# DRL-Navigation/DDRL4NAV

Hardware: AMD Instinct MI355X
Metric: env-steps/sec (whole node) + PPO update ms, Pong 256 envs at 1/2/4/8 GPUs (higher is better)
Workload: dtype f32 (f16x3 MFMA planes, fp32 accumulate)

## Files before the change

ddrl4nav_amd/csrc/common.h:

```cpp
#pragma once
#include <hip/hip_runtime.h>
#include <stdint.h>

#include "../../include/ddrl.h"

namespace ddrl {

constexpr int IMG = 84;
constexpr int FEAT = 512;
constexpr int FLAT = 3136;
constexpr int C1_OC = 32, C1_KS = 8, C1_S = 4, C1_OW = 20, C1_P = 400;
constexpr int C2_IC = 32, C2_OC = 64, C2_KS = 4, C2_S = 2, C2_IW = 20, C2_OW = 9, C2_P = 81, C2_K = 512;
constexpr int C3_IC = 64, C3_OC = 64, C3_KS = 3, C3_S = 1, C3_IW = 9, C3_OW = 7, C3_P = 49, C3_K = 576;
constexpr float LEAKY = 0.01f;

struct EncLayout {
  int64_t c1w, c1b, c2w, c2b, c3w, c3b, lw, lb, size;
};
struct ParamLayout {
  int A, C;
  int NE;
  EncLayout enc;
  int64_t enc_base[2];
  int64_t actor_w, actor_b, critic_w, critic_b;
  int64_t n_params, n_actor;
};

inline ParamLayout make_layout(int A, int C, bool shared = false) {
  ParamLayout L;
  L.A = A;
  L.C = C;
  L.NE = shared ? 1 : 2;
  int64_t o = 0;
  L.enc.c1w = o; o += (int64_t)C1_OC * C * 64;
  L.enc.c1b = o; o += C1_OC;
  L.enc.c2w = o; o += (int64_t)C2_OC * C2_K;
  L.enc.c2b = o; o += C2_OC;
  L.enc.c3w = o; o += (int64_t)C3_OC * C3_K;
  L.enc.c3b = o; o += C3_OC;
  L.enc.lw = o; o += (int64_t)FEAT * FLAT;
  L.enc.lb = o; o += FEAT;
  L.enc.size = o;
  int64_t p = 0;
  L.enc_base[0] = p; p += L.enc.size;
  L.actor_w = p; p += (int64_t)A * FEAT;
  L.actor_b = p; p += A;
  L.n_actor = p;
  L.critic_w = p; p += FEAT;
  L.critic_b = p; p += 1;
  if (shared) {
    L.enc_base[1] = L.enc_base[0];
    L.n_params = p;
    L.n_actor = p;
    return L;
  }
  L.enc_base[1] = p; p += L.enc.size;
  L.n_params = p;
  return L;
}

struct Workspace {
  unsigned short* wp1b;
  unsigned short* wp2b;
  unsigned short* wp3b;
  unsigned short* wd2b;
  unsigned short* wd3b;
  unsigned short* wlb;
  unsigned short* wdlb;
  float* amax;
  float* actmax;
  float *a1, *a2, *a3, *h;
  unsigned* m1;
  unsigned* m2;
  unsigned* m3;
  float *dz1, *dz2, *dz3, *dh;
  float* gsc;
  float* dlogits;
  float* dvalue;
  float* wpart;
  int64_t wpart_floats;
  float* hpart;
  double* npart;
  float* lut;
  int64_t total_bytes;
};

constexpr int AMAX_WL = 0, AMAX_W2 = 1, AMAX_W3 = 2, AMAX_W1 = 3, AMAX_A1 = 4, AMAX_A2 = 5, AMAX_A3 = 6, AMAX_DH = 7, AMAX_DZ3 = 8,
              AMAX_DZ2 = 9, AMAX_DZ1 = 10, AMAX_GMAX = 11, AMAX_SLOTS = 12, AMAX_FIRST_ACT = AMAX_A2;
constexpr float WGRAD_HEADROOM = 4.0f;
constexpr int GSC_EXP_MIN = -60, GSC_EXP_MAX = 60;
__host__ __device__ inline int amax_idx(int slot, int e) { return slot * 2 + e; }
__host__ __device__ inline float f16_scale(float m) {
  if (!(m > 0.0f) || !(m < 3.0e38f)) return 1.0f;
  int e;
  frexpf(m, &e);
  return ldexpf(1.0f, 13 - e);
}
constexpr int HEAD_WG = 256;
constexpr int NORM_WG = 1024;

inline int64_t align_up(int64_t x, int64_t a) { return (x + a - 1) / a * a; }
__host__ __device__ inline int64_t m1_words(int64_t max_batch) { return max_batch * 400; }
__host__ __device__ inline int m1_bit(int oc) { return ((oc >> 2) & 1) * 16 + 15 - ((oc & 3) + 4 * (oc >> 3)); }

constexpr int ACT_FUSED_MAX = 512;
constexpr int FC_ACT_SPLITS = 14;
static_assert(FC_ACT_SPLITS > 1 && 98 % FC_ACT_SPLITS == 0, "FC_ACT_SPLITS: a divisor of 98 larger than 1");
struct Splits {
  int c1, c2, c3, fc;
};
inline Splits choose_splits(int max_batch, int NE = 2) {
  constexpr int C1_SPLITS = 512, C2_SPLITS = 256, C3_SPLITS = 256;
  const int pairs = (max_batch + 1) / 2;
  auto cap = [&](int want, int limit) { return want < limit ? (want < 1 ? 1 : want) : (limit < 1 ? 1 : limit); };
  Splits s;
  s.c1 = cap(C1_SPLITS, pairs);
  const int k = 2 / NE;
  s.c2 = cap(C2_SPLITS * k, pairs);
  s.c3 = cap(C3_SPLITS * k, pairs);
  s.fc = cap(5 * k, (max_batch + 31) / 32);
  return s;
}

inline int64_t hpart_stride(int A) { return align_up((int64_t)(A + 1) * FEAT + A + 1 + 4, 64); }

inline int64_t carve(Workspace& w, const ddrl_config& c, void* base) {
  const int64_t MB = c.max_batch, C = c.in_channels, A = c.n_actions;
  int64_t off = 0;
  auto take = [&](int64_t floats) -> float* {
    float* p = base ? (float*)((char*)base + off) : nullptr;
    off += align_up(floats * 4, 256);
    return p;
  };
  w.wp1b = (unsigned short*)take(4 * 4 * 3 * 2 * 64 * 8 / 2);
  w.wlb = (unsigned short*)take(2 * 3 * (int64_t)FLAT * FEAT / 2);
  w.wdlb = (unsigned short*)take(2 * 3 * (int64_t)FLAT * FEAT / 2);
  w.amax = take(64);
  w.actmax = take(2 * ACT_FUSED_MAX);
  w.wp2b = (unsigned short*)take(2 * 32 * 3 * 64 * 16 / 2);
  w.wp3b = (unsigned short*)take(2 * 8 * 5 * 3 * 64 * 16 / 2);
  w.wd2b = (unsigned short*)take(2 * 2 * 4 * 4 * 3 * 64 * 16 / 2);
  w.wd3b = (unsigned short*)take(2 * 8 * 5 * 3 * 64 * 16 / 2);
  w.a1 = take(2 * MB * 32 * 400);
  w.m1 = (unsigned*)take(2 * m1_words(MB));
  w.m2 = (unsigned*)take(2 * MB * 81 * 2);
  w.m3 = (unsigned*)take(2 * MB * 49 * 2);
  w.a2 = take(2 * MB * 64 * 81);
  w.a3 = take(2 * MB * FLAT);
  w.h = take(2 * MB * FEAT);
  w.dz1 = take(2 * MB * 32 * 400);
  w.dz2 = take(2 * MB * 64 * 81);
  w.dz3 = take(2 * MB * FLAT);
  w.dh = take(2 * MB * FEAT);
  w.gsc = take(2 * MB);
  w.dlogits = take(MB * A);
  w.dvalue = take(MB);
  Splits s = choose_splits(c.max_batch, c.share_cnn_net ? 1 : 2);
  int64_t p1 = (int64_t)s.c1 * 2 * (32 * C * 64 + 32);
  int64_t p2 = (int64_t)s.c2 * 2 * (64 * 512 + 64);
  int64_t p3 = (int64_t)s.c3 * 2 * (64 * 576 + 64);
  int64_t pf = (int64_t)s.fc * 2 * ((int64_t)FEAT * FLAT + FEAT);
  int64_t pm = p1;
  if (p2 > pm) pm = p2;
  if (p3 > pm) pm = p3;
  if (pf > pm) pm = pf;
  const int64_t pact = (int64_t)FC_ACT_SPLITS * 2 * (MB < 1024 ? MB : 1024) * FEAT;
  if (pact > pm) pm = pact;
  w.wpart_floats = pm;
  w.wpart = take(pm);
  w.hpart = take((int64_t)HEAD_WG * hpart_stride(A));
  w.npart = (double*)take(NORM_WG * 2);
  w.lut = take(256);
  w.total_bytes = off;
  return off;
}

__host__ __device__ inline uint64_t splitmix64(uint64_t x) {
  x += 0x9E3779B97F4A7C15ull;
  uint64_t z = x;
  z = (z ^ (z >> 30)) * 0xBF58476D1CE4E5B9ull;
  z = (z ^ (z >> 27)) * 0x94D049BB133111EBull;
  return z ^ (z >> 31);
}
__host__ __device__ inline float hash_uniform(uint64_t seed, uint64_t stream, uint64_t idx) {
  uint64_t base = splitmix64(splitmix64(seed) ^ stream);
  uint64_t z = splitmix64(base + idx);
  return (float)(z >> 40) * (1.0f / 16777216.0f);
}

}
```

ddrl4nav_amd/csrc/conv2.hip:

```cpp
#include "engine2.h"

namespace ddrl {


using u4v = __attribute__((ext_vector_type(4))) unsigned;

constexpr int F1_PITCH = 168;
template <int NE>
struct Fwd1B {
  static constexpr int ROWS = 32 * NE, A_BYTES = 4 * NPL * 2 * ROWS * 16, PITCH = F1_PITCH, IMG_BYTES = 64 * PITCH;
  static constexpr int STAGE_BYTES = A_BYTES + IMG_BYTES, AQ = A_BYTES / 16, NAJ = AQ / 256;
  static constexpr size_t LDS_BYTES = 2 * STAGE_BYTES;
};

template <int NE>
__global__ __launch_bounds__(256) void conv_fwd1_planes_kernel(const uint8_t* __restrict__ frames, const unsigned short* __restrict__ wp1b,
                                                               float* __restrict__ amax, const float* __restrict__ params, int64_t bias_off0,
                                                               int64_t bias_off1, float* __restrict__ out, int64_t out_es, int n,
                                                               unsigned* __restrict__ m1, int64_t m1_es, int C) {
  using K = Fwd1B<NE>;
  extern __shared__ __attribute__((aligned(16))) char ldsb[];
  const int tid = threadIdx.x, lane = tid & 63, wc = tid >> 6, l31 = lane & 31, hi = lane >> 5;
  const int c0 = blockIdx.x * 256, ctot = n * 400, clast = min(c0 + 255, ctot - 1);
  const int b0 = c0 / 400, b1 = clast / 400, oyf0 = (c0 % 400) / 20, iy0_start = 4 * oyf0;
// ... 289 lines not shown
                     w.wp1b, w.amax, c.params, L.enc_base[0] + L.enc.c1b, L.enc_base[NE - 1] + L.enc.c1b, w.a1, c.max_batch * 12800, c.n,
                     acting ? (unsigned*)nullptr : w.m1, m1_words(c.max_batch), L.C);
}

struct Fwd2B {
  static constexpr int SPT = 3, KC = 2;
  static constexpr int WPE = 3;
  static constexpr int ROW = 52, CH = 20 * ROW, IMG_PLANE = SPT * KC * CH;
  static constexpr int W_OFF = NPL * IMG_PLANE, W_BYTES = KC * NPL * 64 * 32;
  static constexpr int BIAS_OFF = W_OFF + W_BYTES;
  static constexpr int NIU = SPT * KC * 100, NIJ = (NIU + 255) / 256;
  static constexpr int NWJ = W_BYTES / 16 / 256;
  static constexpr int STAGE_BYTES = BIAS_OFF;
  static constexpr size_t LDS_BYTES = STAGE_BYTES + 64 * 4;
};
struct __attribute__((packed, aligned(4))) lds_u2 {
  unsigned x, y;
};

__global__ __launch_bounds__(256) __attribute__((amdgpu_waves_per_eu(Fwd2B::WPE, Fwd2B::WPE))) void conv_fwd2_planes_kernel(const float* __restrict__ a1, int64_t a1_es, const unsigned short* __restrict__ wp2b,
                                                               float* __restrict__ amax, const float* __restrict__ params, int64_t bias_off0,
                                                               int64_t bias_off1, float* __restrict__ out, int64_t out_es, int n,
                                                               unsigned* __restrict__ m2) {
  using K = Fwd2B;
  extern __shared__ __attribute__((aligned(16))) char ldsc2[];
  const int tid = threadIdx.x, lane = tid & 63, wc = tid >> 6, l31 = lane & 31, hi = lane >> 5;
  const int e = blockIdx.z, b0 = blockIdx.x * K::SPT;
  const float sa = plane_scale(amax[amax_idx(AMAX_A1, e)]), inv = 1.0f / (sa * plane_scale(amax[amax_idx(AMAX_W2, e)]));
  if (tid < 64) ((float*)(ldsc2 + K::STAGE_BYTES))[tid] = params[(e ? bias_off1 : bias_off0) + tid];
  const float* isrc[K::NIJ];
  int idst[K::NIJ];
#pragma unroll
  for (int j = 0; j < K::NIJ; ++j) {
    const int u = min(tid + 256 * j, K::NIU - 1);
    const int s = u / (100 * K::KC), rem = u % (100 * K::KC), q = rem % 100;
    isrc[j] = a1 + e * a1_es + (int64_t)min(b0 + s, n - 1) * 12800 + rem * 4;
    idst[j] = (s * K::KC + rem / 100) * K::CH + (q / 5) * K::ROW + (q % 5) * 8;
  }
  const unsigned short* wsrc = wp2b + (int64_t)e * (32 * NPL * 64 * 16) + tid * 8;
  int aA[2], bB[2];
#pragma unroll
  for (int i = 0; i < 2; ++i) aA[i] = K::W_OFF + (i * 32 + l31) * 32 + hi * 16;
#pragma unroll
  for (int j = 0; j < 2; ++j) {
    int c = wc * 64 + j * 32 + l31;
    if (c >= K::SPT * 81) c = 0;
    const int s = c / 81, pix = c % 81, oy = pix / 9, ox = pix % 9;
    bB[j] = s * K::KC * K::CH + (2 * oy + 2 * hi) * K::ROW + 4 * ox;
  }
  f4 ir[K::NIJ], wr[K::NWJ];
  auto fetch = [&](int kb) {
#pragma unroll
    for (int j = 0; j < K::NIJ; ++j) ir[j] = ld4(isrc[j] + kb * (400 * K::KC));
#pragma unroll
    for (int j = 0; j < K::NWJ; ++j) wr[j] = *(const f4*)(wsrc + kb * (K::KC * NPL * 1024) + j * 2048);
  };
  auto commit = [&](char* ldsc2) {
#pragma unroll
    for (int j = 0; j < K::NIJ; ++j) {
      if (j + 1 < K::NIJ || tid + 256 * j < K::NIU) {
        const f4 v = ir[j];
        unsigned pa[NPL], pb[NPL];
        split_planes(v.x, v.y, sa, pa);
        split_planes(v.z, v.w, sa, pb);
        char* d = ldsc2 + idst[j];
#pragma unroll
        for (int p = 0; p < NPL; ++p) *(lds_u2*)(d + p * K::IMG_PLANE) = lds_u2{pa[p], pb[p]};
      }
    }
#pragma unroll
    for (int j = 0; j < K::NWJ; ++j) *(f4*)(ldsc2 + K::W_OFF + (tid + 256 * j) * 16) = wr[j];
  };
  f32x16 acc[2][2];
#pragma unroll
  for (int i = 0; i < 2; ++i)
#pragma unroll
    for (int j = 0; j < 2; ++j)
#pragma unroll
      for (int r = 0; r < 16; ++r) acc[i][j][r] = 0.0f;
  constexpr int NKB = 32 / K::KC;
  auto compute = [&](const char* ldsc2) {
#pragma unroll
    for (int kg = 0; kg < K::KC; ++kg) {
      frag8 a[NPL][2], b[NPL][2];
#pragma unroll
      for (int p = 0; p < NPL; ++p) {
#pragma unroll
        for (int i = 0; i < 2; ++i) a[p][i] = *(const frag8*)(ldsc2 + aA[i] + (kg * NPL + p) * 2048);
#pragma unroll
        for (int j = 0; j < 2; ++j) {
          const char* q = ldsc2 + bB[j] + p * K::IMG_PLANE + kg * K::CH;
          const lds_u2 lo = *(const lds_u2*)q, up = *(const lds_u2*)(q + K::ROW);
          b[p][j] = __builtin_bit_cast(frag8, (u4v){lo.x, lo.y, up.x, up.y});
        }
      }
#pragma unroll
      for (int t = 0; t < NPROD; ++t)
#pragma unroll
        for (int i = 0; i < 2; ++i)
#pragma unroll
          for (int j = 0; j < 2; ++j) acc[i][j] = mfma_planes(a[PA[t]][i], b[PB[t]][j], acc[i][j]);
    }
  };
  fetch(0);
  commit(ldsc2);
  fetch(1);
  __syncthreads();
  for (int kb = 0; kb < NKB; ++kb) {
    compute(ldsc2);
    __syncthreads();
    if (kb + 1 < NKB) {
      commit(ldsc2);
      if (kb + 2 < NKB) fetch(kb + 2);
    }
    __syncthreads();
  }
  const float* bias = (const float*)(ldsc2 + K::STAGE_BYTES);
  float big = 0.0f;
#pragma unroll
  for (int j = 0; j < 2; ++j) {
    const int c = wc * 64 + j * 32 + l31;
    const int s = c / 81, pix = c % 81;
    if (c >= K::SPT * 81 || b0 + s >= n) continue;
    float* base = out + e * out_es + (int64_t)b0 * 5184;
    const uint32_t lb = (uint32_t)((s * 5184 + pix + hi * (4 * 81)) * 4);
    unsigned bits = 0u;
#pragma unroll
    for (int i = 0; i < 2; ++i)
#pragma unroll
      for (int r = 0; r < 16; ++r) {
        const int oc = i * 32 + acc_row(r, hi);
        const float y = leaky_f(__builtin_fmaf(acc[i][j][r], inv, bias[oc]));
        st1_so(base + (i * 32 + acc_row(r, 0)) * 81, lb, y);
        big = fmaxf(big, fabsf(y));
        bits = __builtin_amdgcn_alignbit(bits, (unsigned)__builtin_elementwise_sub_sat((int)__float_as_uint(y), 1), 31);
      }
    if (m2 != nullptr) m2[(e * (out_es / 5184) + b0 + s) * 162 + pix * 2 + hi] = (bits >> 16) | (bits << 16);
  }
  amax_update(big, amax + amax_idx(AMAX_A2, e));
}
static void launch_fwd2_planes(const EncCall& c, bool acting, hipStream_t st) {
  using K = Fwd2B;
  const Workspace& w = *c.ws;
  const ParamLayout& L = *c.L;
  lds_limit_once<conv_fwd2_planes_kernel>((int)K::LDS_BYTES);
  hipLaunchKernelGGL(conv_fwd2_planes_kernel, dim3((unsigned)((c.n + K::SPT - 1) / K::SPT), 1, (unsigned)L.NE), dim3(256), K::LDS_BYTES, st, w.a1,
                     c.max_batch * 12800, w.wp2b, w.amax, c.params, L.enc_base[0] + L.enc.c2b, L.enc_base[L.NE - 1] + L.enc.c2b, w.a2, c.max_batch * 5184,
                     c.n, acting ? (unsigned*)nullptr : w.m2);
}

struct Fwd3B {
  static constexpr int WPE = 3;
  static constexpr int TN = 2, SPT = (128 * TN) / 49, NPX = SPT * 81;
  static constexpr int IMG_PLANE = NPX * 16;
  static constexpr int W_OFF = NPL * IMG_PLANE, W_BYTES = 5 * NPL * 64 * 32;
  static constexpr int BIAS_OFF = W_OFF + W_BYTES;
  static constexpr int NIJ = (NPX + 255) / 256;
  static constexpr int NWJ = (W_BYTES / 16 + 255) / 256;
  static constexpr size_t LDS_BYTES = BIAS_OFF + 64 * 4;
};

__global__ __launch_bounds__(256) __attribute__((amdgpu_waves_per_eu(Fwd3B::WPE, Fwd3B::WPE))) void conv_fwd3_planes_kernel(const float* __restrict__ a2, int64_t a2_es, const unsigned short* __restrict__ wp3b,
                                                               float* __restrict__ amax, const float* __restrict__ params, int64_t bias_off0,
                                                               int64_t bias_off1, float* __restrict__ out, int64_t out_es, int n,
                                                               unsigned* __restrict__ m3) {
  using K = Fwd3B;
  extern __shared__ __attribute__((aligned(16))) char ldsc3[];
  const int tid = threadIdx.x, lane = tid & 63, wc = tid >> 6, l31 = lane & 31, hi = lane >> 5;
  const int e = blockIdx.z, b0 = blockIdx.x * K::SPT;
  const float sa = plane_scale(amax[amax_idx(AMAX_A2, e)]), inv = 1.0f / (sa * plane_scale(amax[amax_idx(AMAX_W3, e)]));
  if (tid < 64) ((float*)(ldsc3 + K::BIAS_OFF))[tid] = params[(e ? bias_off1 : bias_off0) + tid];
  const float* isrc[K::NIJ];
#pragma unroll
  for (int j = 0; j < K::NIJ; ++j) {
    const int u = min(tid + 256 * j, K::NPX - 1);
    const int s = u / 81, px = u % 81;
    isrc[j] = a2 + e * a2_es + (int64_t)min(b0 + s, n - 1) * 5184 + px;
  }
  const unsigned short* wsrc = wp3b + (int64_t)e * (8 * 5 * NPL * 64 * 16) + tid * 8;
  int aA[2], bB[K::TN], tapoff[5];
#pragma unroll
  for (int i = 0; i < 2; ++i) aA[i] = K::W_OFF + (i * 32 + l31) * 32 + hi * 16;
#pragma unroll
  for (int j = 0; j < K::TN; ++j) {
    int c = wc * (32 * K::TN) + j * 32 + l31;
    if (c >= K::SPT * 49) c = 0;
    const int s = c / 49, pix = c % 49;
    bB[j] = (s * 81 + (pix / 7) * 9 + pix % 7) * 16;
  }
#pragma unroll
  for (int kg = 0; kg < 5; ++kg) {
    const int tap = min(2 * kg + hi, 8);
    tapoff[kg] = ((tap / 3) * 9 + tap % 3) * 16;
  }
  float ir[K::NIJ][8];
  f4 wr[K::NWJ];
  auto fetch = [&](int kb) {
#pragma unroll
    for (int j = 0; j < K::NIJ; ++j)
#pragma unroll
      for (int c = 0; c < 8; ++c) ir[j][c] = isrc[j][(kb * 8 + c) * 81];
#pragma unroll
    for (int j = 0; j < K::NWJ; ++j)
      if (j + 1 < K::NWJ || tid + 256 * j < K::W_BYTES / 16) wr[j] = *(const f4*)(wsrc + kb * (5 * NPL * 1024) + j * 2048);
  };
  auto commit = [&]() {
#pragma unroll
    for (int j = 0; j < K::NIJ; ++j) {
      if (j + 1 < K::NIJ || tid + 256 * j < K::NPX) {
        unsigned pl[4][NPL];
#pragma unroll
        for (int c = 0; c < 4; ++c) split_planes(ir[j][2 * c], ir[j][2 * c + 1], sa, pl[c]);
        char* d = ldsc3 + (tid + 256 * j) * 16;
#pragma unroll
        for (int p = 0; p < NPL; ++p) *(u4v*)(d + p * K::IMG_PLANE) = (u4v){pl[0][p], pl[1][p], pl[2][p], pl[3][p]};
      }
    }
#pragma unroll
    for (int j = 0; j < K::NWJ; ++j)
      if (j + 1 < K::NWJ || tid + 256 * j < K::W_BYTES / 16) *(f4*)(ldsc3 + K::W_OFF + (tid + 256 * j) * 16) = wr[j];
  };
  f32x16 acc[2][K::TN];
#pragma unroll
  for (int i = 0; i < 2; ++i)
#pragma unroll
    for (int j = 0; j < K::TN; ++j)
#pragma unroll
      for (int r = 0; r < 16; ++r) acc[i][j][r] = 0.0f;
  constexpr int NKB = 8;
  fetch(0);
  commit();
  fetch(1);
  __syncthreads();
  for (int kb = 0; kb < NKB; ++kb) {
#pragma unroll
    for (int kg = 0; kg < 5; ++kg) {
      frag8 a[NPL][2], b[NPL][K::TN];
#pragma unroll
      for (int p = 0; p < NPL; ++p) {
#pragma unroll
        for (int i = 0; i < 2; ++i) a[p][i] = *(const frag8*)(ldsc3 + aA[i] + (kg * NPL + p) * 2048);
#pragma unroll
        for (int j = 0; j < K::TN; ++j) b[p][j] = *(const frag8*)(ldsc3 + bB[j] + tapoff[kg] + p * K::IMG_PLANE);
      }
#pragma unroll
      for (int t = 0; t < NPROD; ++t)
#pragma unroll
        for (int i = 0; i < 2; ++i)
#pragma unroll
          for (int j = 0; j < K::TN; ++j) acc[i][j] = mfma_planes(a[PA[t]][i], b[PB[t]][j], acc[i][j]);
    }
    __syncthreads();
    if (kb + 1 < NKB) {
      commit();
      if (kb + 2 < NKB) fetch(kb + 2);
    }
    __syncthreads();
  }
  const float* bias = (const float*)(ldsc3 + K::BIAS_OFF);
  float big = 0.0f;
#pragma unroll
  for (int j = 0; j < K::TN; ++j) {
    const int c = wc * (32 * K::TN) + j * 32 + l31;
    const int s = c / 49, pix = c % 49;
    if (c >= K::SPT * 49 || b0 + s >= n) continue;
    float* base = out + e * out_es + (int64_t)b0 * FLAT;
    const uint32_t lb = (uint32_t)((s * FLAT + pix + hi * (4 * 49)) * 4);
    unsigned bits = 0u;
#pragma unroll
    for (int i = 0; i < 2; ++i)
#pragma unroll
      for (int r = 0; r < 16; ++r) {
        const int oc = i * 32 + acc_row(r, hi);
        const float y = leaky_f(__builtin_fmaf(acc[i][j][r], inv, bias[oc]));
        st1_so(base + (i * 32 + acc_row(r, 0)) * 49, lb, y);
        big = fmaxf(big, fabsf(y));
        bits = __builtin_amdgcn_alignbit(bits, (unsigned)__builtin_elementwise_sub_sat((int)__float_as_uint(y), 1), 31);
      }
    if (m3 != nullptr) m3[(e * (out_es / FLAT) + b0 + s) * 98 + pix * 2 + hi] = (bits >> 16) | (bits << 16);
  }
  amax_update(big, amax + amax_idx(AMAX_A3, e));
}
static void launch_fwd3_planes(const EncCall& c, bool acting, hipStream_t st) {
  using K = Fwd3B;
  const Workspace& w = *c.ws;
  const ParamLayout& L = *c.L;
  lds_limit_once<conv_fwd3_planes_kernel>((int)K::LDS_BYTES);
  hipLaunchKernelGGL(conv_fwd3_planes_kernel, dim3((unsigned)((c.n + K::SPT - 1) / K::SPT), 1, (unsigned)L.NE), dim3(256), K::LDS_BYTES, st, w.a2,
                     c.max_batch * 5184, w.wp3b, w.amax, c.params, L.enc_base[0] + L.enc.c3b, L.enc_base[L.NE - 1] + L.enc.c3b, w.a3, c.max_batch * FLAT,
                     c.n, acting ? (unsigned*)nullptr : w.m3);
}


void launch_conv_forward2(const EncCall& c, bool acting, hipStream_t st) {
  {
    ProfRange pr(c.prof, acting ? "ConvFwd1.act" : "ConvFwd1", st);
    if (c.L->NE == 2) {
      launch_fwd1_planes<2>(c, acting, st);
    } else {
      launch_fwd1_planes<1>(c, acting, st);
    }
  }
  {
    ProfRange pr(c.prof, acting ? "ConvFwd2.act" : "ConvFwd2", st);
    launch_fwd2_planes(c, acting, st);
  }
  {
    ProfRange pr(c.prof, acting ? "ConvFwd3.act" : "ConvFwd3", st);
    launch_fwd3_planes(c, acting, st);
  }
}

struct Dgrad3B {
  static constexpr int THREADS = 256, TN = 2, SPT = ((THREADS / 64) * 32 * TN) / 81;
  static constexpr int KOC = 16, NKB = 64 / KOC, PIXB = 2 * KOC;
  static constexpr int IMG_PLANE = SPT * 121 * PIXB;
  static constexpr int W_OFF = NPL * IMG_PLANE, W_BYTES = 9 * NPL * 64 * 32;
  static constexpr int NIU = SPT * 49, NIJ = (NIU + THREADS - 1) / THREADS;
  static constexpr int NWQ = W_BYTES / 16, NWJ = (NWQ + THREADS - 1) / THREADS;
  static constexpr size_t LDS_BYTES = W_OFF + W_BYTES;
};

__global__ __launch_bounds__(Dgrad3B::THREADS) __attribute__((amdgpu_waves_per_eu(2, 2))) void conv_dgrad3_planes_kernel(
    const float* __restrict__ dz3, int64_t dz_es, const unsigned short* __restrict__ wd3b, float* __restrict__ amax, const unsigned* __restrict__ m2,
    float* __restrict__ out, int64_t out_es, int n) {
  using K = Dgrad3B;
  extern __shared__ __attribute__((aligned(16))) char ldsd3[];
  const int tid = threadIdx.x, lane = tid & 63, wc = tid >> 6, l31 = lane & 31, hi = lane >> 5;
  const int e = blockIdx.z, b0 = blockIdx.x * K::SPT;
  const float sa = plane_scale(amax[amax_idx(AMAX_DZ3, e)]), inv = 1.0f / (sa * plane_scale(amax[amax_idx(AMAX_W3, e)]));
  for (int i = tid; i < K::W_OFF / 16; i += K::THREADS) *(f4*)(ldsd3 + i * 16) = zero4();
  const float* isrc[K::NIJ];
  int idst[K::NIJ];
#pragma unroll
  for (int j = 0; j < K::NIJ; ++j) {
    const int u = min(tid + K::THREADS * j, K::NIU - 1);
    const int s = u / 49, px = u % 49;
    isrc[j] = dz3 + e * dz_es + (int64_t)min(b0 + s, n - 1) * FLAT + px;
    idst[j] = (s * 121 + (px / 7 + 2) * 11 + px % 7 + 2) * K::PIXB;
  }
  const unsigned short* wsrc = wd3b + (int64_t)e * (K::NKB * 9 * NPL * 64 * 16) + tid * 8;
  int aA[2], bB[K::TN];
#pragma unroll
  for (int i = 0; i < 2; ++i) aA[i] = K::W_OFF + (i * 32 + l31) * 32 + hi * 16;
#pragma unroll
  for (int j = 0; j < K::TN; ++j) {
    int c = wc * (32 * K::TN) + j * 32 + l31;
    if (c >= K::SPT * 81) c = 0;
    const int s = c / 81, pix = c % 81;
    bB[j] = (s * 121 + (pix / 9 + 2) * 11 + pix % 9 + 2) * K::PIXB + hi * 16;
  }
  float ir[K::NIJ][K::KOC];
  f4 wr[K::NWJ];
  auto fetch = [&](int kb) {
#pragma unroll
    for (int j = 0; j < K::NIJ; ++j)
#pragma unroll
      for (int c = 0; c < K::KOC; ++c) ir[j][c] = isrc[j][(kb * K::KOC + c) * 49];
#pragma unroll
    for (int j = 0; j < K::NWJ; ++j)
      if (j + 1 < K::NWJ || tid + K::THREADS * j < K::NWQ) wr[j] = *(const f4*)(wsrc + kb * (9 * NPL * 1024) + j * (K::THREADS * 8));
  };
  auto commit = [&]() {
#pragma unroll
    for (int j = 0; j < K::NIJ; ++j) {
      if (j + 1 < K::NIJ || tid + K::THREADS * j < K::NIU) {
        unsigned pl[K::KOC / 2][NPL];
#pragma unroll
        for (int c = 0; c < K::KOC / 2; ++c) split_planes(ir[j][2 * c], ir[j][2 * c + 1], sa, pl[c]);
        char* d = ldsd3 + idst[j];
#pragma unroll
        for (int p = 0; p < NPL; ++p) {
          *(u4v*)(d + p * K::IMG_PLANE) = (u4v){pl[0][p], pl[1][p], pl[2][p], pl[3][p]};
          *(u4v*)(d + p * K::IMG_PLANE + 16) = (u4v){pl[4][p], pl[5][p], pl[6][p], pl[7][p]};
        }
      }
    }
#pragma unroll
    for (int j = 0; j < K::NWJ; ++j)
      if (j + 1 < K::NWJ || tid + K::THREADS * j < K::NWQ) *(f4*)(ldsd3 + K::W_OFF + (tid + K::THREADS * j) * 16) = wr[j];
  };
  f32x16 acc[2][K::TN];
#pragma unroll
  for (int i = 0; i < 2; ++i)
#pragma unroll
    for (int j = 0; j < K::TN; ++j)
#pragma unroll
      for (int r = 0; r < 16; ++r) acc[i][j][r] = 0.0f;
  fetch(0);
  __syncthreads();
  commit();
  fetch(1);
  __syncthreads();
  for (int kb = 0; kb < K::NKB; ++kb) {
#pragma unroll
    for (int t = 0; t < 9; ++t) {
      constexpr int ROW11 = 11;
      const int toff = ((t / 3) * ROW11 + t % 3) * K::PIXB;
      frag8 af[NPL][2], bfr[NPL][K::TN];
#pragma unroll
      for (int p = 0; p < NPL; ++p) {
#pragma unroll
        for (int i = 0; i < 2; ++i) af[p][i] = *(const frag8*)(ldsd3 + aA[i] + (t * NPL + p) * 2048);
#pragma unroll
        for (int j = 0; j < K::TN; ++j) bfr[p][j] = *(const frag8*)(ldsd3 + bB[j] - toff + p * K::IMG_PLANE);
      }
#pragma unroll
      for (int m = 0; m < NPROD; ++m)
#pragma unroll
        for (int i = 0; i < 2; ++i)
#pragma unroll
          for (int j = 0; j < K::TN; ++j) acc[i][j] = mfma_planes(af[PA[m]][i], bfr[PB[m]][j], acc[i][j]);
    }
    __syncthreads();
    if (kb + 1 < K::NKB) {
      commit();
      if (kb + 2 < K::NKB) fetch(kb + 2);
    }
    __syncthreads();
  }
  float big = 0.0f;
#pragma unroll
  for (int j = 0; j < K::TN; ++j) {
    const int c = wc * (32 * K::TN) + j * 32 + l31;
    const int s = c / 81, pix = c % 81;
    if (c >= K::SPT * 81 || b0 + s >= n) continue;
    const int64_t off = (int64_t)(b0 + s) * 5184 + pix + hi * (4 * 81);
    float* op = out + e * out_es + off;
    const unsigned mw = m2[(e * (out_es / 5184) + b0 + s) * 162 + pix * 2 + hi];
#pragma unroll
    for (int i = 0; i < 2; ++i)
#pragma unroll
      for (int r = 0; r < 16; ++r) {
        const float g = leaky_bit(mw, 16 * i + 15 - r, acc[i][j][r] * inv);
        op[(i * 32 + acc_row(r, 0)) * 81] = g;
        big = fmaxf(big, fabsf(g));
      }
  }
  amax_update(big, amax + amax_idx(AMAX_DZ2, e));
}
static void launch_dgrad3_planes(const EncCall& c, hipStream_t st) {
  using K = Dgrad3B;
// ... 137 lines not shown
```

ddrl4nav_amd/csrc/optim.hip:

```cpp
#include "engine2.h"

namespace ddrl {

__device__ __forceinline__ void pack_conv1_planes_body(const float* __restrict__ params, const ParamLayout& L, unsigned short* __restrict__ dst,
                                                       const float* __restrict__ amax, int bx) {
  const int rows = 32 * L.NE;
  const int idx = bx * 256 + threadIdx.x;
  if (idx >= L.C * 4 * 2 * rows * 8) return;
  const int j = idx & 7, row = (idx >> 3) % rows, r = (idx >> 3) / rows;
  const int h = r & 1, g = (r >> 1) & 3, c = r >> 3;
  const int e = row >> 5, oc = row & 31, ky = 2 * g + h;
  const float w = params[L.enc_base[e] + L.enc.c1w + ((oc * L.C + c) * 8 + ky) * 8 + j];
  unsigned short pl[NPL];
  planes_of(w, plane_scale(amax[amax_idx(AMAX_W1, e)]), pl);
  const int base = (c * 4 + g) * NPL;
#pragma unroll
  for (int p = 0; p < NPL; ++p) dst[(((base + p) * 2 + h) * rows + row) * 8 + j] = pl[p];
}

__device__ __forceinline__ void pack_fc_planes_body(const float* __restrict__ params, const ParamLayout& L, unsigned short* __restrict__ dst,
                                                    unsigned short* __restrict__ dst_t, const float* __restrict__ amax,
                                                    unsigned short (&tile)[NPL][32][33], int bx, int by, int e) {
  const int k0 = bx * 32, n0 = by * 32;
  const int tx = threadIdx.x & 31, ty = threadIdx.x >> 5;
  const float sc = plane_scale(amax[amax_idx(AMAX_WL, e)]);
  const float* src = params + L.enc_base[e] + L.enc.lw;
  unsigned short* d = dst + (int64_t)e * 3 * FLAT * FEAT;
  unsigned short* t = dst_t + (int64_t)e * 3 * FLAT * FEAT;
#pragma unroll
  for (int j = 0; j < 4; ++j) {
    const int n = n0 + ty + 8 * j, k = k0 + tx;
    unsigned short pl[NPL];
    planes_of(src[(int64_t)n * FLAT + k], sc, pl);
#pragma unroll
    for (int p = 0; p < NPL; ++p) {
      d[p * (int64_t)FLAT * FEAT + (int64_t)n * FLAT + k] = pl[p];
      tile[p][ty + 8 * j][tx] = pl[p];
    }
  }
  __syncthreads();
#pragma unroll
  for (int j = 0; j < 4; ++j) {
    const int k = k0 + ty + 8 * j, n = n0 + tx;
#pragma unroll
    for (int p = 0; p < NPL; ++p) t[p * (int64_t)FLAT * FEAT + (int64_t)k * FEAT + n] = tile[p][tx][ty + 8 * j];
  }
}

__device__ __forceinline__ void pack_conv2_planes_body(const float* __restrict__ params, const ParamLayout& L, unsigned short* __restrict__ dst, const float* __restrict__ amax, int bx, int e) {
  const int i = bx * 256 + threadIdx.x;
  if (i >= 64 * 32 * 16) return;
  const int tap = i & 15, ch = (i >> 4) & 31, oc = i >> 9;
  const float w = params[L.enc_base[e] + L.enc.c2w + i];
  unsigned short pl[NPL];
  planes_of(w, plane_scale(amax[amax_idx(AMAX_W2, e)]), pl);
  unsigned short* d = dst + (((int64_t)(e * 32 + ch) * NPL) * 64 + oc) * 16 + tap;
#pragma unroll
  for (int p = 0; p < NPL; ++p) d[p * 64 * 16] = pl[p];
}

__device__ __forceinline__ void pack_conv3_planes_body(const float* __restrict__ params, const ParamLayout& L, unsigned short* __restrict__ dst, const float* __restrict__ amax, int bx, int e) {
  const int i = bx * 256 + threadIdx.x;
  if (i >= 8 * 5 * 64 * 16) return;
  const int c = i & 7, h = (i >> 3) & 1, oc = (i >> 4) & 63, kg = (i >> 10) % 5, kb = (i >> 10) / 5;
  const int tap = 2 * kg + h;
  const float w = tap < 9 ? params[L.enc_base[e] + L.enc.c3w + (oc * 64 + kb * 8 + c) * 9 + tap] : 0.0f;
  unsigned short pl[NPL];
  planes_of(w, plane_scale(amax[amax_idx(AMAX_W3, e)]), pl);
  unsigned short* d = dst + ((((int64_t)(e * 8 + kb) * 5 + kg) * NPL) * 64 + oc) * 16 + h * 8 + c;
#pragma unroll
  for (int p = 0; p < NPL; ++p) d[p * 64 * 16] = pl[p];
}

__device__ __forceinline__ void pack_dgrad2_planes_body(const float* __restrict__ params, const ParamLayout& L, unsigned short* __restrict__ dst, const float* __restrict__ amax, int bx, int e) {
  const int i = bx * 256 + threadIdx.x;
  if (i >= 2 * 8 * 2 * 64 * 16) return;
  const int o = i & 7, v = (i >> 3) & 1, row = (i >> 4) & 63, u = (i >> 10) & 1, kb = (i >> 11) & 7, a = i >> 14;
  const int c = row >> 5, ic = row & 31, oc = 8 * kb + o;
  const float w = params[L.enc_base[e] + L.enc.c2w + (oc * 32 + ic) * 16 + (2 * u + a) * 4 + 2 * v + c];
  unsigned short pl[NPL];
  planes_of(w, plane_scale(amax[amax_idx(AMAX_W2, e)]), pl);
  unsigned short* d = dst + (((((int64_t)(e * 2 + a) * 8 + kb) * 2 + u) * NPL) * 64 + row) * 16 + v * 8 + o;
#pragma unroll
  for (int p = 0; p < NPL; ++p) d[p * 64 * 16] = pl[p];
}

__device__ __forceinline__ void pack_dgrad3_planes_body(const float* __restrict__ params, const ParamLayout& L, unsigned short* __restrict__ dst, const float* __restrict__ amax, int bx, int e) {
  const int i = bx * 256 + threadIdx.x;
  if (i >= 4 * 9 * 64 * 16) return;
  const int o = i & 7, h = (i >> 3) & 1, ic = (i >> 4) & 63, tap = (i >> 10) % 9, kb = (i >> 10) / 9;
  const float w = params[L.enc_base[e] + L.enc.c3w + ((16 * kb + 8 * h + o) * 64 + ic) * 9 + tap];
  unsigned short pl[NPL];
  planes_of(w, plane_scale(amax[amax_idx(AMAX_W3, e)]), pl);
  unsigned short* d = dst + ((((int64_t)(e * 4 + kb) * 9 + tap) * NPL) * 64 + ic) * 16 + h * 8 + o;
#pragma unroll
  for (int p = 0; p < NPL; ++p) d[p * 64 * 16] = pl[p];
}

constexpr int WA_NBLK[4] = {128, 8, 8, 4};
constexpr int WA_BLOCKS = 128 + 8 + 8 + 4, A1B_BLOCKS = 8;
__global__ __launch_bounds__(256) void weights_amax_kernel(const float* __restrict__ params, ParamLayout L, float* __restrict__ amax) {
  int bid = blockIdx.x;
  if (bid >= WA_BLOCKS * L.NE) {
    bid -= WA_BLOCKS * L.NE;
    const int e = bid / A1B_BLOCKS, oc = (bid % A1B_BLOCKS) * 4 + (threadIdx.x >> 6), lane = threadIdx.x & 63, K = L.C * 64;
    const float* wsrc = params + L.enc_base[e] + L.enc.c1w + (int64_t)oc * K;
    float s = 0.0f;
    for (int k = lane; k < K; k += 64) s += fabsf(wsrc[k]);
#pragma unroll
    for (int off = 32; off >= 1; off >>= 1) s += __shfl_xor(s, off, 64);
    amax_update(s + fabsf(params[L.enc_base[e] + L.enc.c1b + oc]), amax + amax_idx(AMAX_A1, e));
    return;
  }
  const int e = bid / WA_BLOCKS;
  int b = bid % WA_BLOCKS, t = 0;
  while (b >= WA_NBLK[t]) b -= WA_NBLK[t], ++t;
  const int nb = WA_NBLK[t];
  const int64_t off = t == AMAX_WL ? L.enc.lw : t == AMAX_W2 ? L.enc.c2w : t == AMAX_W3 ? L.enc.c3w : L.enc.c1w;
  const int64_t cnt = t == AMAX_WL ? (int64_t)FEAT * FLAT : t == AMAX_W2 ? (int64_t)C2_OC * C2_K : t == AMAX_W3 ? (int64_t)C3_OC * C3_K
                                                                                                              : (int64_t)C1_OC * L.C * 64;
  const float* src = params + L.enc_base[e] + off;
  float m = 0.0f;
  const int64_t stride = (int64_t)nb * 256;
  int64_t i = (int64_t)b * 256 + threadIdx.x;
  for (; i + 7 * stride < cnt; i += 8 * stride) {
    float x[8];
#pragma unroll
    for (int u = 0; u < 8; ++u) x[u] = src[i + u * stride];
#pragma unroll
    for (int u = 0; u < 8; ++u) m = fmaxf(m, fabsf(x[u]));
  }
  for (; i < cnt; i += stride) m = fmaxf(m, fabsf(src[i]));
  __shared__ float wm[4];
  m = wave_fmax(m);
  if ((threadIdx.x & 63) == 0) wm[threadIdx.x >> 6] = m;
  __syncthreads();
  if (threadIdx.x == 0) atomicMax((unsigned*)(amax + amax_idx(t, e)), __float_as_uint(fmaxf(fmaxf(wm[0], wm[1]), fmaxf(wm[2], wm[3]))));
}

constexpr int PK_D3 = 4 * 9 * 64 * 16 / 256, PK_D2 = 2 * 8 * 2 * 64 * 16 / 256, PK_C3 = 8 * 5 * 64 * 16 / 256, PK_C2 = 64 * 32 * 16 / 256;
constexpr int PK_FC = (FLAT / 32) * (FEAT / 32);
static_assert(FLAT % 32 == 0 && FEAT % 32 == 0, "whole 32 x 32 tiles");
__global__ __launch_bounds__(256) void pack_all_planes_kernel(const float* __restrict__ params, ParamLayout L, unsigned short* __restrict__ wd3b,
                                                             unsigned short* __restrict__ wd2b, unsigned short* __restrict__ wp3b,
                                                             unsigned short* __restrict__ wp2b, unsigned short* __restrict__ wlb,
                                                             unsigned short* __restrict__ wdlb, unsigned short* __restrict__ wp1b,
                                                             const float* __restrict__ amax) {
  __shared__ unsigned short tile[NPL][32][33];
  int b = blockIdx.x;
  const int ne = L.NE;
  if (b < PK_FC * ne) {
    const int e = b / PK_FC, r = b % PK_FC;
    pack_fc_planes_body(params, L, wlb, wdlb, amax, tile, r % (FLAT / 32), r / (FLAT / 32), e);
    return;
  }
  b -= PK_FC * ne;
  if (b < PK_D3 * ne) return pack_dgrad3_planes_body(params, L, wd3b, amax, b % PK_D3, b / PK_D3);
  b -= PK_D3 * ne;
  if (b < PK_D2 * ne) return pack_dgrad2_planes_body(params, L, wd2b, amax, b % PK_D2, b / PK_D2);
  b -= PK_D2 * ne;
  if (b < PK_C3 * ne) return pack_conv3_planes_body(params, L, wp3b, amax, b % PK_C3, b / PK_C3);
  b -= PK_C3 * ne;
  if (b < PK_C2 * ne) return pack_conv2_planes_body(params, L, wp2b, amax, b % PK_C2, b / PK_C2);
  b -= PK_C2 * ne;
  pack_conv1_planes_body(params, L, wp1b, amax, b);
}

void launch_pack_weights(const Workspace& w, const ParamLayout& L, const float* params, hipStream_t st) {
  static_assert(AMAX_WL == 0 && AMAX_W2 == 1 && AMAX_W3 == 2 && AMAX_W1 == 3 && AMAX_A1 == 4 && AMAX_FIRST_ACT == 5,
                "weight slots and the bound of a1 come first");
  (void)hipMemsetAsync(w.amax, 0, AMAX_FIRST_ACT * 2 * sizeof(float), st);
  hipLaunchKernelGGL(weights_amax_kernel, dim3((WA_BLOCKS + A1B_BLOCKS) * L.NE), dim3(256), 0, st, params, L, w.amax);
  const int c1_blocks = (L.C * 4 * 2 * 32 * L.NE * 8 + 255) / 256;
  hipLaunchKernelGGL(pack_all_planes_kernel, dim3((PK_FC + PK_D3 + PK_D2 + PK_C3 + PK_C2) * L.NE + c1_blocks), dim3(256), 0, st, params, L,
                     w.wd3b, w.wd2b, w.wp3b, w.wp2b, w.wlb, w.wdlb, w.wp1b, w.amax);
}

__global__ __launch_bounds__(256) void reduce_partials_kernel(const float* __restrict__ part, int nsplit, int64_t count,
                                                              float* __restrict__ grads, int64_t off0, int64_t off1) {
  const int e = blockIdx.y;
  const int64_t i = (int64_t)blockIdx.x * 256 + threadIdx.x;
  if (i >= count) return;
  double s = 0.0;
  int sp = 0;
  for (; sp + 8 <= nsplit; sp += 8) {
    float x[8];
#pragma unroll
    for (int t = 0; t < 8; ++t) x[t] = part[((int64_t)(sp + t) * 2 + e) * count + i];
#pragma unroll
    for (int t = 0; t < 8; ++t) s += (double)x[t];
  }
  for (; sp < nsplit; ++sp) s += (double)part[((int64_t)sp * 2 + e) * count + i];
  grads[(e ? off1 : off0) + i] = (float)s;
}
__global__ __launch_bounds__(256) void reduce_partials_wide_kernel(const float* __restrict__ part, int nsplit, int64_t count,
                                                                   float* __restrict__ grads, int64_t off0, int64_t off1) {
  __shared__ double red[16][17];
  const int e = blockIdx.y;
  const int el = threadIdx.x & 15, g = threadIdx.x >> 4;
  const int64_t i = (int64_t)blockIdx.x * 16 + el;
  double s = 0.0;
  if (i < count)
    for (int sp = g; sp < nsplit; sp += 16) s += (double)part[((int64_t)sp * 2 + e) * count + i];
  red[g][el] = s;
  __syncthreads();
  if (g == 0 && i < count) {
    double t = 0.0;
#pragma unroll
    for (int q = 0; q < 16; ++q) t += red[q][el];
    grads[(e ? off1 : off0) + i] = (float)t;
  }
}
void launch_reduce_partials(const float* part, int nsplit, int64_t count, int ne, float* grads, int64_t off0,
                            int64_t off1, hipStream_t st) {
  if (nsplit >= 64 && count < 65536)
    hipLaunchKernelGGL(reduce_partials_wide_kernel, dim3((unsigned)((count + 15) / 16), ne), dim3(256), 0, st, part, nsplit,
                       count, grads, off0, off1);
  else
    hipLaunchKernelGGL(reduce_partials_kernel, dim3((unsigned)((count + 255) / 256), ne), dim3(256), 0, st, part, nsplit,
                       count, grads, off0, off1);
}

__global__ __launch_bounds__(256) void sqnorm_kernel(const float* __restrict__ g, int64_t n, double* __restrict__ part) {
  __shared__ double red[256];
  double s = 0.0;
  for (int64_t i = (int64_t)blockIdx.x * 256 + threadIdx.x; i < n; i += (int64_t)gridDim.x * 256) {
    const double x = (double)g[i];
    s += x * x;
  }
  red[threadIdx.x] = s;
  __syncthreads();
  for (int off = 128; off > 0; off >>= 1) {
    if (threadIdx.x < off) red[threadIdx.x] += red[threadIdx.x + off];
    __syncthreads();
  }
  if (threadIdx.x == 0) part[blockIdx.x] = red[0];
}

struct AdamArgs {
  float lr_step[2];
  float bc2_sqrt;
  float beta1, beta2, eps;
  float max_norm;
  int clip;
  float v_theta, ent_theta;
};

__global__ __launch_bounds__(256) void clip_adam_kernel(float* __restrict__ p, float* __restrict__ g, float* __restrict__ m,
                                                        float* __restrict__ v, int64_t n, int64_t n_actor,
                                                        const double* __restrict__ part, int nparts, AdamArgs a) {
  __shared__ float s_coef;
  if (threadIdx.x < 64) {
    double s = 0.0;
    for (int i = threadIdx.x; i < nparts; i += 64) s += part[i];
#pragma unroll
    for (int off = 32; off >= 1; off >>= 1) s += __shfl_xor(s, off, 64);
    if (threadIdx.x == 0) {
      const float norm = (float)sqrt(s);
      float coef = a.max_norm / (norm + 1e-6f);
      coef = fminf(coef, 1.0f);
      if (!a.clip) coef = 1.0f;
      s_coef = coef;
      if (blockIdx.x == 0) {
        g[n + 4] = norm;
        g[n + 5] = coef;
        g[n + 3] = g[n + 0] + g[n + 1] * a.v_theta - g[n + 2] * a.ent_theta;
      }
    }
  }
  __syncthreads();
  const float coef = s_coef;
  for (int64_t i = (int64_t)blockIdx.x * 256 + threadIdx.x; i < n; i += (int64_t)gridDim.x * 256) {
    const float gi = g[i] * coef;
    float mi = m[i], vi = v[i];
    mi = mi + (gi - mi) * (1.0f - a.beta1);
    vi = vi * a.beta2 + ((1.0f - a.beta2) * gi) * gi;
    const float denom = sqrtf(vi) / a.bc2_sqrt + a.eps;
    const float step = (i < n_actor) ? a.lr_step[0] : a.lr_step[1];
    p[i] = p[i] + (-step) * (mi / denom);
    m[i] = mi;
    v[i] = vi;
    g[i] = gi;
  }
}

void launch_clip_adam(const ddrl_config& cfg, const ParamLayout& L, const Workspace& w, float* params, float* grads,
                      float* m, float* v, int64_t step, hipStream_t st) {
  hipLaunchKernelGGL(sqnorm_kernel, dim3(NORM_WG), dim3(256), 0, st, grads, L.n_params, w.npart);
  AdamArgs a;
  const double bc1 = 1.0 - pow((double)cfg.adam_beta1, (double)step);
  const double bc2 = 1.0 - pow((double)cfg.adam_beta2, (double)step);
  if (L.NE == 1) {
    a.lr_step[0] = a.lr_step[1] = (float)((double)cfg.learning_rate / bc1);
  } else {
    a.lr_step[0] = (float)((double)cfg.actor_lr / bc1);
    a.lr_step[1] = (float)((double)cfg.critic_lr / bc1);
  }
  a.bc2_sqrt = (float)sqrt(bc2);
  a.beta1 = cfg.adam_beta1;
  a.beta2 = cfg.adam_beta2;
  a.eps = cfg.adam_eps;
  a.max_norm = cfg.clip_grad_norm;
  a.clip = cfg.clip_grad;
  a.v_theta = cfg.v_loss_theta;
  a.ent_theta = cfg.ent_loss_theta;
  hipLaunchKernelGGL(clip_adam_kernel, dim3(2048), dim3(256), 0, st, params, grads, m, v, L.n_params, L.n_actor, w.npart,
                     NORM_WG, a);
}

__global__ __launch_bounds__(64) void gae_kernel(const float* __restrict__ values, const float* __restrict__ rewards,
                                                 const uint8_t* __restrict__ dones, int T, int N, float gamma, float landa,
                                                 float* __restrict__ adv, float* __restrict__ ret) {
  const int n = blockIdx.x * 64 + threadIdx.x;
  if (n >= N) return;
  const float gl = __fmul_rn(gamma, landa);
  float g = 0.0f;
  float nv = values[(int64_t)T * N + n];
#pragma unroll 8
  for (int t = T - 1; t >= 0; --t) {
    const int64_t i = (int64_t)t * N + n;
    const float d = (float)(uint8_t)(1 - dones[i]);
    const float v = values[i];
    const float r = rewards[i];
    g = __fmul_rn(g, d);
    const float t1 = __fmul_rn(gl, g);
    const float t2 = __fmul_rn(__fmul_rn(gamma, nv), d);
    const float t3 = __fadd_rn(__fsub_rn(t2, v), r);
    g = __fadd_rn(t1, t3);
// ... 43 lines not shown
```

Baseline: 257,400.

## Pair conv3 k-blocks to drop padded tap and double-buffer image tiles

The conv3 forward kernel used to handle 8 k-blocks of 9 taps as 5 k-groups each, with the last group padded by clamping tap 8, which wasted MFMA work. It now processes k-blocks in pairs as 9 k-groups, with the two tap-8 halves merged into one group, using a new weight packing (wp3f) and two LDS image buffers. This removes the redundant padded MFMAs, giving 36 k-groups instead of 40. In exchange it adds a pack pass, more workspace, a larger LDS footprint under the WPE=3 occupancy constraint, and extra barriers per iteration.

New measurement: 258,300, median of 6. About the same (+0.4%).

```diff
diff --git a/ddrl4nav_amd/csrc/common.h b/ddrl4nav_amd/csrc/common.h
--- a/ddrl4nav_amd/csrc/common.h
+++ b/ddrl4nav_amd/csrc/common.h
@@ -63,6 +63,7 @@
   unsigned short* wp1b;
   unsigned short* wp2b;
   unsigned short* wp3b;
+  unsigned short* wp3f;
   unsigned short* wd2b;
   unsigned short* wd3b;
   unsigned short* wlb;
@@ -139,6 +140,7 @@
   w.actmax = take(2 * ACT_FUSED_MAX);
   w.wp2b = (unsigned short*)take(2 * 32 * 3 * 64 * 16 / 2);
   w.wp3b = (unsigned short*)take(2 * 8 * 5 * 3 * 64 * 16 / 2);
+  w.wp3f = (unsigned short*)take(2 * 4 * 9 * 3 * 64 * 16 / 2);
   w.wd2b = (unsigned short*)take(2 * 2 * 4 * 4 * 3 * 64 * 16 / 2);
   w.wd3b = (unsigned short*)take(2 * 8 * 5 * 3 * 64 * 16 / 2);
   w.a1 = take(2 * MB * 32 * 400);
diff --git a/ddrl4nav_amd/csrc/conv2.hip b/ddrl4nav_amd/csrc/conv2.hip
--- a/ddrl4nav_amd/csrc/conv2.hip
+++ b/ddrl4nav_amd/csrc/conv2.hip
@@ -465,15 +465,17 @@
 struct Fwd3B {
   static constexpr int WPE = 3;
   static constexpr int TN = 2, SPT = (128 * TN) / 49, NPX = SPT * 81;
-  static constexpr int IMG_PLANE = NPX * 16;
-  static constexpr int W_OFF = NPL * IMG_PLANE, W_BYTES = 5 * NPL * 64 * 32;
+  static constexpr int IMG_PLANE = NPX * 16, IMG_BUF = NPL * IMG_PLANE;
+  static constexpr int KG_BYTES = NPL * 64 * 32;
+  static constexpr int W_OFF = 2 * IMG_BUF, W_BYTES = 5 * KG_BYTES;
   static constexpr int BIAS_OFF = W_OFF + W_BYTES;
   static constexpr int NIJ = (NPX + 255) / 256;
-  static constexpr int NWJ = (W_BYTES / 16 + 255) / 256;
   static constexpr size_t LDS_BYTES = BIAS_OFF + 64 * 4;
+  static_assert(KG_BYTES == 256 * 16, "one 16-byte quad per thread and k-group");
+  static_assert(WPE * LDS_BYTES <= 160 * 1024, "WPE workgroups share the CU's LDS");
 };
 
-__global__ __launch_bounds__(256) __attribute__((amdgpu_waves_per_eu(Fwd3B::WPE, Fwd3B::WPE))) void conv_fwd3_planes_kernel(const float* __restrict__ a2, int64_t a2_es, const unsigned short* __restrict__ wp3b,
+__global__ __launch_bounds__(256) __attribute__((amdgpu_waves_per_eu(Fwd3B::WPE, Fwd3B::WPE))) void conv_fwd3_planes_kernel(const float* __restrict__ a2, int64_t a2_es, const unsigned short* __restrict__ wp3f,
                                                                float* __restrict__ amax, const float* __restrict__ params, int64_t bias_off0,
                                                                int64_t bias_off1, float* __restrict__ out, int64_t out_es, int n,
                                                                unsigned* __restrict__ m3) {
@@ -490,8 +492,8 @@
     const int s = u / 81, px = u % 81;
     isrc[j] = a2 + e * a2_es + (int64_t)min(b0 + s, n - 1) * 5184 + px;
   }
-  const unsigned short* wsrc = wp3b + (int64_t)e * (8 * 5 * NPL * 64 * 16) + tid * 8;
-  int aA[2], bB[K::TN], tapoff[5];
+  const unsigned short* wsrc = wp3f + (int64_t)e * (4 * 9 * NPL * 1024) + tid * 8;
+  int aA[2], bB[K::TN], tapoff[4];
 #pragma unroll
   for (int i = 0; i < 2; ++i) aA[i] = K::W_OFF + (i * 32 + l31) * 32 + hi * 16;
 #pragma unroll
@@ -502,36 +504,37 @@
     bB[j] = (s * 81 + (pix / 7) * 9 + pix % 7) * 16;
   }
 #pragma unroll
-  for (int kg = 0; kg < 5; ++kg) {
-    const int tap = min(2 * kg + hi, 8);
+  for (int kg = 0; kg < 4; ++kg) {
+    const int tap = 2 * kg + hi;
     tapoff[kg] = ((tap / 3) * 9 + tap % 3) * 16;
   }
+  const int tap8off = hi * K::IMG_BUF + (2 * 9 + 2) * 16;
   float ir[K::NIJ][8];
-  f4 wr[K::NWJ];
-  auto fetch = [&](int kb) {
+  f4 wr[5];
+  auto fetch = [&](auto odd, int kb) {
+    constexpr int ODD = decltype(odd)::value;
 #pragma unroll
     for (int j = 0; j < K::NIJ; ++j)
 #pragma unroll
       for (int c = 0; c < 8; ++c) ir[j][c] = isrc[j][(kb * 8 + c) * 81];
 #pragma unroll
-    for (int j = 0; j < K::NWJ; ++j)
-      if (j + 1 < K::NWJ || tid + 256 * j < K::W_BYTES / 16) wr[j] = *(const f4*)(wsrc + kb * (5 * NPL * 1024) + j * 2048);
-  };
-  auto commit = [&]() {
+    for (int j = 0; j < 4 + ODD; ++j) wr[j] = *(const f4*)(wsrc + ((kb >> 1) * 9 + 4 * ODD + j) * (NPL * 1024));
+  };
+  auto commit = [&](auto odd) {
+    constexpr int ODD = decltype(odd)::value;
 #pragma unroll
     for (int j = 0; j < K::NIJ; ++j) {
       if (j + 1 < K::NIJ || tid + 256 * j < K::NPX) {
         unsigned pl[4][NPL];
 #pragma unroll
         for (int c = 0; c < 4; ++c) split_planes(ir[j][2 * c], ir[j][2 * c + 1], sa, pl[c]);
-        char* d = ldsc3 + (tid + 256 * j) * 16;
+        char* d = ldsc3 + ODD * K::IMG_BUF + (tid + 256 * j) * 16;
 #pragma unroll
         for (int p = 0; p < NPL; ++p) *(u4v*)(d + p * K::IMG_PLANE) = (u4v){pl[0][p], pl[1][p], pl[2][p], pl[3][p]};
       }
     }
 #pragma unroll
-    for (int j = 0; j < K::NWJ; ++j)
-      if (j + 1 < K::NWJ || tid + 256 * j < K::W_BYTES / 16) *(f4*)(ldsc3 + K::W_OFF + (tid + 256 * j) * 16) = wr[j];
+    for (int j = 0; j < 4 + ODD; ++j) *(f4*)(ldsc3 + K::W_OFF + (tid + 256 * j) * 16) = wr[j];
   };
   f32x16 acc[2][K::TN];
 #pragma unroll
@@ -540,33 +543,44 @@
     for (int j = 0; j < K::TN; ++j)
 #pragma unroll
       for (int r = 0; r < 16; ++r) acc[i][j][r] = 0.0f;
-  constexpr int NKB = 8;
-  fetch(0);
-  commit();
-  fetch(1);
+  auto compute = [&](auto odd) {
+    constexpr int ODD = decltype(odd)::value;
+#pragma unroll
+    for (int kg = 0; kg < 4 + ODD; ++kg) {
+      const int boff = kg < 4 ? ODD * K::IMG_BUF + tapoff[kg & 3] : tap8off;
+      frag8 a[NPL][2], b[NPL][K::TN];
+#pragma unroll
+      for (int p = 0; p < NPL; ++p) {
+#pragma unroll
+        for (int i = 0; i < 2; ++i) a[p][i] = *(const frag8*)(ldsc3 + aA[i] + (kg * NPL + p) * 2048);
+#pragma unroll
+        for (int j = 0; j < K::TN; ++j) b[p][j] = *(const frag8*)(ldsc3 + bB[j] + boff + p * K::IMG_PLANE);
+      }
+#pragma unroll
+      for (int t = 0; t < NPROD; ++t)
+#pragma unroll
+        for (int i = 0; i < 2; ++i)
+#pragma unroll
+          for (int j = 0; j < K::TN; ++j) acc[i][j] = mfma_planes(a[PA[t]][i], b[PB[t]][j], acc[i][j]);
+    }
+  };
+  constexpr std::integral_constant<int, 0> EVEN{};
+  constexpr std::integral_constant<int, 1> ODDB{};
+  fetch(EVEN, 0);
+  commit(EVEN);
+  fetch(ODDB, 1);
   __syncthreads();
-  for (int kb = 0; kb < NKB; ++kb) {
-#pragma unroll
-    for (int kg = 0; kg < 5; ++kg) {
-      frag8 a[NPL][2], b[NPL][K::TN];
-#pragma unroll
-      for (int p = 0; p < NPL; ++p) {
-#pragma unroll
-        for (int i = 0; i < 2; ++i) a[p][i] = *(const frag8*)(ldsc3 + aA[i] + (kg * NPL + p) * 2048);
-#pragma unroll
-        for (int j = 0; j < K::TN; ++j) b[p][j] = *(const frag8*)(ldsc3 + bB[j] + tapoff[kg] + p * K::IMG_PLANE);
-      }
-#pragma unroll
-      for (int t = 0; t < NPROD; ++t)
-#pragma unroll
-        for (int i = 0; i < 2; ++i)
-#pragma unroll
-          for (int j = 0; j < K::TN; ++j) acc[i][j] = mfma_planes(a[PA[t]][i], b[PB[t]][j], acc[i][j]);
-    }
-    __syncthreads();
-    if (kb + 1 < NKB) {
-      commit();
-      if (kb + 2 < NKB) fetch(kb + 2);
+  for (int m = 0; m < 4; ++m) {
+    compute(EVEN);
+    __syncthreads();
+    commit(ODDB);
+    if (m < 3) fetch(EVEN, 2 * m + 2);
+    __syncthreads();
+    compute(ODDB);
+    __syncthreads();
+    if (m < 3) {
+      commit(EVEN);
+      fetch(ODDB, 2 * m + 3);
     }
     __syncthreads();
   }
@@ -600,7 +614,7 @@
   const ParamLayout& L = *c.L;
   lds_limit_once<conv_fwd3_planes_kernel>((int)K::LDS_BYTES);
   hipLaunchKernelGGL(conv_fwd3_planes_kernel, dim3((unsigned)((c.n + K::SPT - 1) / K::SPT), 1, (unsigned)L.NE), dim3(256), K::LDS_BYTES, st, w.a2,
-                     c.max_batch * 5184, w.wp3b, w.amax, c.params, L.enc_base[0] + L.enc.c3b, L.enc_base[L.NE - 1] + L.enc.c3b, w.a3, c.max_batch * FLAT,
+                     c.max_batch * 5184, w.wp3f, w.amax, c.params, L.enc_base[0] + L.enc.c3b, L.enc_base[L.NE - 1] + L.enc.c3b, w.a3, c.max_batch * FLAT,
                      c.n, acting ? (unsigned*)nullptr : w.m3);
 }
 
diff --git a/ddrl4nav_amd/csrc/optim.hip b/ddrl4nav_amd/csrc/optim.hip
--- a/ddrl4nav_amd/csrc/optim.hip
+++ b/ddrl4nav_amd/csrc/optim.hip
@@ -68,6 +68,19 @@
   unsigned short pl[NPL];
   planes_of(w, plane_scale(amax[amax_idx(AMAX_W3, e)]), pl);
   unsigned short* d = dst + ((((int64_t)(e * 8 + kb) * 5 + kg) * NPL) * 64 + oc) * 16 + h * 8 + c;
+#pragma unroll
+  for (int p = 0; p < NPL; ++p) d[p * 64 * 16] = pl[p];
+}
+
+__device__ __forceinline__ void pack_conv3_pairs_body(const float* __restrict__ params, const ParamLayout& L, unsigned short* __restrict__ dst, const float* __restrict__ amax, int bx, int e) {
+  const int i = bx * 256 + threadIdx.x;
+  if (i >= 4 * 9 * 64 * 16) return;
+  const int c = i & 7, h = (i >> 3) & 1, oc = (i >> 4) & 63, kg = (i >> 10) % 9, m = (i >> 10) / 9;
+  const int kb = kg < 8 ? 2 * m + (kg >> 2) : 2 * m + h, tap = kg < 8 ? 2 * (kg & 3) + h : 8;
+  const float w = params[L.enc_base[e] + L.enc.c3w + (oc * 64 + kb * 8 + c) * 9 + tap];
+  unsigned short pl[NPL];
+  planes_of(w, plane_scale(amax[amax_idx(AMAX_W3, e)]), pl);
+  unsigned short* d = dst + ((((int64_t)(e * 4 + m) * 9 + kg) * NPL) * 64 + oc) * 16 + h * 8 + c;
 #pragma unroll
   for (int p = 0; p < NPL; ++p) d[p * 64 * 16] = pl[p];
 }
@@ -138,12 +151,12 @@
   if (threadIdx.x == 0) atomicMax((unsigned*)(amax + amax_idx(t, e)), __float_as_uint(fmaxf(fmaxf(wm[0], wm[1]), fmaxf(wm[2], wm[3]))));
 }
 
-constexpr int PK_D3 = 4 * 9 * 64 * 16 / 256, PK_D2 = 2 * 8 * 2 * 64 * 16 / 256, PK_C3 = 8 * 5 * 64 * 16 / 256, PK_C2 = 64 * 32 * 16 / 256;
+constexpr int PK_D3 = 4 * 9 * 64 * 16 / 256, PK_D2 = 2 * 8 * 2 * 64 * 16 / 256, PK_C3 = 8 * 5 * 64 * 16 / 256, PK_C3F = 4 * 9 * 64 * 16 / 256, PK_C2 = 64 * 32 * 16 / 256;
 constexpr int PK_FC = (FLAT / 32) * (FEAT / 32);
 static_assert(FLAT % 32 == 0 && FEAT % 32 == 0, "whole 32 x 32 tiles");
 __global__ __launch_bounds__(256) void pack_all_planes_kernel(const float* __restrict__ params, ParamLayout L, unsigned short* __restrict__ wd3b,
                                                              unsigned short* __restrict__ wd2b, unsigned short* __restrict__ wp3b,
-                                                             unsigned short* __restrict__ wp2b, unsigned short* __restrict__ wlb,
+                                                             unsigned short* __restrict__ wp3f, unsigned short* __restrict__ wp2b, unsigned short* __restrict__ wlb,
                                                              unsigned short* __restrict__ wdlb, unsigned short* __restrict__ wp1b,
                                                              const float* __restrict__ amax) {
   __shared__ unsigned short tile[NPL][32][33];
@@ -161,6 +174,8 @@
   b -= PK_D2 * ne;
   if (b < PK_C3 * ne) return pack_conv3_planes_body(params, L, wp3b, amax, b % PK_C3, b / PK_C3);
   b -= PK_C3 * ne;
+  if (b < PK_C3F * ne) return pack_conv3_pairs_body(params, L, wp3f, amax, b % PK_C3F, b / PK_C3F);
+  b -= PK_C3F * ne;
   if (b < PK_C2 * ne) return pack_conv2_planes_body(params, L, wp2b, amax, b % PK_C2, b / PK_C2);
   b -= PK_C2 * ne;
   pack_conv1_planes_body(params, L, wp1b, amax, b);
@@ -172,8 +187,8 @@
   (void)hipMemsetAsync(w.amax, 0, AMAX_FIRST_ACT * 2 * sizeof(float), st);
   hipLaunchKernelGGL(weights_amax_kernel, dim3((WA_BLOCKS + A1B_BLOCKS) * L.NE), dim3(256), 0, st, params, L, w.amax);
   const int c1_blocks = (L.C * 4 * 2 * 32 * L.NE * 8 + 255) / 256;
-  hipLaunchKernelGGL(pack_all_planes_kernel, dim3((PK_FC + PK_D3 + PK_D2 + PK_C3 + PK_C2) * L.NE + c1_blocks), dim3(256), 0, st, params, L,
-                     w.wd3b, w.wd2b, w.wp3b, w.wp2b, w.wlb, w.wdlb, w.wp1b, w.amax);
+  hipLaunchKernelGGL(pack_all_planes_kernel, dim3((PK_FC + PK_D3 + PK_D2 + PK_C3 + PK_C3F + PK_C2) * L.NE + c1_blocks), dim3(256), 0, st, params, L,
+                     w.wd3b, w.wd2b, w.wp3b, w.wp3f, w.wp2b, w.wlb, w.wdlb, w.wp1b, w.amax);
 }
 
 __global__ __launch_bounds__(256) void reduce_partials_kernel(const float* __restrict__ part, int nsplit, int64_t count,
```
